# ilya16/MultINN

Measured on AMD Instinct MI355X. Metric: piano-roll timesteps/sec (train step), 5-track LSTM-NADE, higher is better.
Workload: dtype fp16; 1 GPU; TGT joint LSTM-NADE [1024,256,88,5]; global_batch=1024, per_gpu_batch=1024, seq_len=256, pitches=88, tracks=5, nade_hidden=256, optimizer=TF-Adam lr 0.01 eps 1e-4 clip 5.0, parallelism=dp1

## Files before the change

multinn_amd/csrc/nade_mfma.hip:

```cpp
#include "common.h"
typedef float nm_f4 __attribute__((ext_vector_type(4)));
#define NM_ST4(dst, a) __builtin_nontemporal_store((nm_f4){a[0], a[1], a[2], a[3]}, reinterpret_cast<nm_f4*>(dst))
#define NM_ST1(dst, x) __builtin_nontemporal_store((float)(x), dst)
#include <algorithm>
#include <type_traits>

typedef __bf16 bf16x8_t __attribute__((ext_vector_type(8)));
typedef float f32x4_t __attribute__((ext_vector_type(4)));
typedef __attribute__((address_space(1))) const void* gas_ptr_t;
typedef __attribute__((address_space(3))) void* lds_ptr_t;

#ifdef NM_TRACE
__device__ long long nm_trace[16];
#define NM_T(k) do { if (tid == 0 && blockIdx.x == NM_TRACE) { const long long now_ = wall_clock64(); nm_trace[k] += now_ - tprev_; tprev_ = now_; } } while (0)
#else
#define NM_T(k) do { } while (0)
#endif
#define NADE_EPS 1e-6f
#define LN2F 0.6931471805599453f
#define NM_H 256
#define NM_PITCH 264
#define NM_LP 36

__device__ __forceinline__ void lds_barrier() { asm volatile("s_waitcnt lgkmcnt(0)\n\ts_barrier" ::: "memory"); }

__device__ __forceinline__ float nm_ln(float x) { return __builtin_amdgcn_logf(x) * LN2F; }

typedef _Float16 f16x8_t __attribute__((ext_vector_type(8)));
struct NmPairB { f16x8_t hi, lo; };
template <bool SPLIT> struct NmState;
template <> struct NmState<false> { typedef bf16_t T; static constexpr int PITCH = NM_PITCH; };
template <> struct NmState<true> { typedef unsigned T; static constexpr int PITCH = 260; };
__device__ __forceinline__ unsigned nm_pack_hl(float x) {
    const float hi = __uint_as_float(__float_as_uint(x) & 0xFFFFE000u);
    return __builtin_bit_cast(unsigned, __builtin_amdgcn_cvt_pkrtz(hi, x - hi));
}

template <bool SPLIT>
struct NadeFwdSmemT {
    float sA[SPLIT ? 1 : 32][NM_H];
    typename NmState<SPLIT>::T sH[32][NmState<SPLIT>::PITCH];
    typename NmState<SPLIT>::T sF[32][NmState<SPLIT>::PITCH];
    float sLb[32][NM_LP];
    float sLf[32][NM_LP];
    unsigned sMask[2][32];
    unsigned sSb[2][33];
    unsigned short sFl[2][1024];
    unsigned short sPs[2][34];
    unsigned sAct[2][32];
};

__device__ __forceinline__ void nm_load_a(const bf16_t (*tile)[NM_PITCH], int mi, int lane, bf16x8_t (&a)[8]) {
    const bf16_t* p = &tile[16 * mi + (lane & 15)][8 * (lane >> 4)];
#pragma unroll
    for (int s = 0; s < 8; ++s) a[s] = *reinterpret_cast<const bf16x8_t*>(p + 32 * s);
}
template <bool SPLIT> __device__ __forceinline__ typename NmState<SPLIT>::T nm_state(float h) {
    if constexpr (SPLIT) return nm_pack_hl(h);
    else return f32_to_bf16(h);
}
__device__ __forceinline__ f32x4_t nm_dot(const bf16x8_t (&af)[8], const bf16x8_t (&bfr)[8]) {
    f32x4_t acc = {0.f, 0.f, 0.f, 0.f};
#pragma unroll
    for (int s = 0; s < 8; ++s) acc = __builtin_amdgcn_mfma_f32_16x16x32_bf16(af[s], bfr[s], acc, 0, 0, 0);
    return acc;
}
__device__ __forceinline__ f32x4_t nm_dot_hl(const unsigned (*tile)[260], int mi, int lane, const NmPairB (&bw)[8]) {
    const unsigned* p = &tile[16 * mi + (lane & 15)][8 * (lane >> 4)];
    f32x4_t accm = {0.f, 0.f, 0.f, 0.f}, accs = {0.f, 0.f, 0.f, 0.f};
#pragma unroll
    for (int s = 0; s < 8; ++s) {
        const uint4 q0 = *reinterpret_cast<const uint4*>(p + 32 * s), q1 = *reinterpret_cast<const uint4*>(p + 32 * s + 4);
        uint4 uh, ul;
        uh.x = __builtin_amdgcn_perm(q0.y, q0.x, 0x05040100u); ul.x = __builtin_amdgcn_perm(q0.y, q0.x, 0x07060302u);
        uh.y = __builtin_amdgcn_perm(q0.w, q0.z, 0x05040100u); ul.y = __builtin_amdgcn_perm(q0.w, q0.z, 0x07060302u);
        uh.z = __builtin_amdgcn_perm(q1.y, q1.x, 0x05040100u); ul.z = __builtin_amdgcn_perm(q1.y, q1.x, 0x07060302u);
        uh.w = __builtin_amdgcn_perm(q1.w, q1.z, 0x05040100u); ul.w = __builtin_amdgcn_perm(q1.w, q1.z, 0x07060302u);
        const f16x8_t ah = __builtin_bit_cast(f16x8_t, uh), al = __builtin_bit_cast(f16x8_t, ul);
        accs = __builtin_amdgcn_mfma_f32_16x16x32_f16(ah, bw[s].lo, accs, 0, 0, 0);
        accm = __builtin_amdgcn_mfma_f32_16x16x32_f16(ah, bw[s].hi, accm, 0, 0, 0);
        accs = __builtin_amdgcn_mfma_f32_16x16x32_f16(al, bw[s].hi, accs, 0, 0, 0);
    }
    return accm + accs;
}
template <bool SPLIT, typename Tile, typename B>
__device__ __forceinline__ void nm_logit_tile(const Tile& tile, int w, int lane, const B& bfr, float (*out)[NM_LP]) {
    const int ni = w >> 1, mi = w & 1;
    f32x4_t acc;
    if constexpr (SPLIT) {
        acc = nm_dot_hl(tile, mi, lane, bfr);
    } else {
        bf16x8_t af[8];
        nm_load_a(tile, mi, lane, af);
        acc = nm_dot(af, bfr);
    }
#pragma unroll
    for (int i = 0; i < 4; ++i) out[16 * mi + 4 * (lane >> 4) + i][16 * ni + (lane & 15)] = acc[i];
}

template <bool SPLIT>
__device__ __forceinline__ void
nade_fwd_mfma_body(int tracks, int N, int D, const uint8_t* __restrict__ v, long v_track_stride, const float* __restrict__ bias, int ld_bias,
                     const float* __restrict__ w_enc, const bf16_t* __restrict__ w_dec_bf, const float* __restrict__ row_weight,
                     float* __restrict__ nll, float* __restrict__ cond_p, float* __restrict__ d_bias, float* __restrict__ a_final,
                     const int* __restrict__ gate, int run_if, const int* __restrict__ n_rows_dev) {
    extern __shared__ __attribute__((aligned(16))) char smem_raw[];
    typedef NadeFwdSmemT<SPLIT> NadeFwdSmem;
    typedef typename NmState<SPLIT>::T state_t;
    typedef typename std::conditional<SPLIT, NmPairB, bf16x8_t>::type bfrag_t;
    constexpr int KS = 8;
    NadeFwdSmem& S = *reinterpret_cast<NadeFwdSmem*>(smem_raw);
    if (gate != nullptr && *gate != run_if) return;
    constexpr int Hn = NM_H;
    const int m = blockIdx.y;
    const int tid = threadIdx.x, lane = tid & 63, w = __builtin_amdgcn_readfirstlane(tid >> 6);
    const int ni = w >> 1;
    const int rb = blockIdx.x * 32;
    const uint8_t* __restrict__ vm = v + (size_t)m * v_track_stride;
    const float* __restrict__ we = w_enc + (size_t)m * D * Hn;
    const bf16_t* __restrict__ wd = w_dec_bf + (size_t)m * D * Hn * (SPLIT ? 2 : 1);
    const int bd_off = tracks * Hn + m * D;
    const int ntile = (D + 31) / 32;
    if (n_rows_dev != nullptr && rb >= *n_rows_dev) {
        if (d_bias != nullptr)
            for (int e = tid; e < 32 * D; e += 256) {
                const int n = e / D, i = e - n * D;
                if (rb + n < N) d_bias[(size_t)(rb + n) * ld_bias + bd_off + i] = 0.f;
            }
        if (nll != nullptr && tid < 32 && rb + tid < N) nll[(size_t)m * N + rb + tid] = 0.f;
        return;
    }

    float areg[SPLIT ? 32 : 1];
    {
        float av[32];
#pragma unroll
        for (int n = 0; n < 32; ++n) av[n] = bias[(size_t)min(rb + n, N - 1) * ld_bias + m * Hn + tid];
#pragma unroll
        for (int n = 0; n < 32; ++n) {
            const float x = rb + n < N ? av[n] : 0.f;
            if constexpr (SPLIT) areg[n] = x;
            else S.sA[n][tid] = x;
            S.sH[n][tid] = nm_state<SPLIT>(fast_sigmoid(x));
        }
    }
    auto load_v = [&](int c, unsigned char (&vb)[4]) {
#pragma unroll
        for (int i = 0; i < 4; ++i) {
            const int row = min(rb + 8 * w + 2 * i + (lane >> 5), N - 1), dd = min(32 * c + (lane & 31), D - 1);
            vb[i] = vm[(size_t)row * D + dd];
        }
    };
    auto ballots = [&](int c, const unsigned char (&vb)[4], unsigned (&msk)[32]) {
#pragma unroll
        for (int i = 0; i < 4; ++i) {
            const int row = rb + 8 * w + 2 * i + (lane >> 5), dd = 32 * c + (lane & 31);
            const unsigned long long bal = __ballot(row < N && dd < D && vb[i] != 0);
            if (lane == 0) { msk[8 * w + 2 * i] = (unsigned)bal; msk[8 * w + 2 * i + 1] = (unsigned)(bal >> 32); }
        }
    };
    auto build_list = [&](int buf) {
        if (w == 0) {
            const unsigned mk = lane < 32 ? S.sMask[buf][lane] : 0u;
            const int cnt = __popc(mk);
            unsigned rest = mk;
            int base = 0;
            for (int j = 0; j < 32; ++j) {
                const unsigned act = (unsigned)__ballot(cnt > j);
                if (lane == 0) { S.sPs[buf][j] = (unsigned short)base; S.sAct[buf][j] = act; }
                if (act == 0u) break;
                if (cnt > j) {
                    const int pos = base + __popc(act & ((1u << lane) - 1u));
                    const int dpos = __builtin_ctz(rest);
                    rest &= rest - 1;
                    S.sFl[buf][pos] = (unsigned short)((lane << 5) | dpos);
                }
                base += __popc(act);
            }
            if (lane == 0) S.sSb[buf][32] = (unsigned)base;
        }
    };
    auto load_b = [&](int c, bfrag_t (&b)[KS]) {
        const int d = min(32 * c + 16 * ni + (lane & 15), D - 1);
        if constexpr (SPLIT) {
            const f16_t* p = reinterpret_cast<const f16_t*>(wd) + (size_t)d * 2 * Hn + 8 * (lane >> 4);
#pragma unroll
            for (int s = 0; s < KS; ++s) {
                b[s].hi = *reinterpret_cast<const f16x8_t*>(p + 32 * s);
                b[s].lo = *reinterpret_cast<const f16x8_t*>(p + Hn + 32 * s);
            }
        } else {
            const bf16_t* p = wd + (size_t)d * Hn + 8 * (lane >> 4);
#pragma unroll
            for (int s = 0; s < KS; ++s) b[s] = *reinterpret_cast<const bf16x8_t*>(p + 32 * s);
        }
    };
    const __amdgpu_buffer_rsrc_t we_rs = __builtin_amdgcn_make_buffer_rsrc(const_cast<float*>(we), 0, D * Hn * 4, 0x00020000);
    auto load_we = [&](int c, int buf, int k0, float (&wv)[32]) {
        const int F = (int)S.sSb[buf][32];
        const int entv = (int)S.sFl[buf][(k0 + (lane & 31) < F) ? k0 + (lane & 31) : 0];
#pragma unroll
        for (int u = 0; u < 32; ++u) {
            const int e = __builtin_amdgcn_readlane(entv, u);
            wv[u] = __builtin_bit_cast(float, __builtin_amdgcn_raw_buffer_load_b32(we_rs, tid * 4, min(32 * c + (e & 31), D - 1) * (Hn * 4), 0));
        }
    };
    unsigned char vb[4];
    bfrag_t bfr[KS];
    float wev[32];
    load_v(0, vb);
    load_b(0, bfr);
    ballots(0, vb, S.sMask[0]);
    if (ntile > 1) load_v(1, vb);
    __syncthreads();
    build_list(0);
    __syncthreads();
    load_we(0, 0, 0, wev);

    const int en = tid >> 3, ed0 = 4 * (tid & 7), erow = rb + en;
    const bool evalid = erow < N;
    const int err = evalid ? erow : N - 1;
    const float rw = (row_weight != nullptr && evalid) ? row_weight[erow] : 0.f;
    float lp = 0.f;
#ifdef NM_TRACE
    long long tprev_ = wall_clock64();
#endif
    for (int c = 0; c < ntile; ++c) {
        const int buf = c & 1, nbuf = buf ^ 1;
        float bdec[4];
        {
            const float* bp = bias + (size_t)err * ld_bias + bd_off + 32 * c + ed0;
            if (32 * c + ed0 + 3 < D && (((size_t)bp) & 15) == 0) {
                const float4 b4 = *reinterpret_cast<const float4*>(bp);
                bdec[0] = b4.x; bdec[1] = b4.y; bdec[2] = b4.z; bdec[3] = b4.w;
            } else {
#pragma unroll
                for (int k = 0; k < 4; ++k) bdec[k] = bias[(size_t)err * ld_bias + bd_off + min(32 * c + ed0 + k, D - 1)];
            }
        }
        __builtin_amdgcn_sched_barrier(0);
        nm_logit_tile<SPLIT>(S.sH, w, lane, bfr, S.sLb);
        if (c + 1 < ntile) {
            ballots(c + 1, vb, S.sMask[nbuf]);
            if (c + 2 < ntile) load_v(c + 2, vb);
        }
        NM_T(0);
        lds_barrier();
        NM_T(1);
        const int F = (int)S.sSb[buf][32];
        const unsigned mk = S.sMask[buf][en];
        float lsel[4];
        int jj[4];
#pragma unroll
        for (int k = 0; k < 4; ++k) {
            jj[k] = __popc(mk & ((1u << (ed0 + k)) - 1u));
            lsel[k] = S.sLb[en][ed0 + k];
        }
        int slot_of[4];
#pragma unroll
        for (int k = 0; k < 4; ++k) {
            const int pj = max(jj[k] - 1, 0);
            slot_of[k] = jj[k] > 0 ? (int)S.sPs[buf][pj] + __popc(S.sAct[buf][pj] & ((1u << en) - 1u)) : -1;
        }
        for (int k0 = 0; k0 < F; k0 += 32) {
            if (k0 > 0) load_we(c, buf, k0, wev);
            const int cnt = min(32, F - k0);
            const int flv = (int)S.sFl[buf][min(k0 + (lane & 31), F - 1)];
#pragma unroll
            for (int u0 = 0; u0 < 32; u0 += 8) {
                if (u0 < cnt) {
                    int n[8];
#pragma unroll
                    for (int i = 0; i < 8; ++i) n[i] = __builtin_amdgcn_readlane(flv, u0 + i) >> 5;
                    if constexpr (SPLIT) {
                        float x[8];
#pragma unroll
                        for (int i = 0; i < 8; ++i) {
                            x[i] = areg[n[i]] + ((u0 + i < cnt) ? wev[u0 + i] : 0.f);
                            areg[n[i]] = x[i];
                        }
                        state_t hb[8];
#pragma unroll
                        for (int i = 0; i < 8; ++i) hb[i] = nm_state<SPLIT>(fast_sigmoid(x[i]));
#pragma unroll
                        for (int i = 0; i < 8; ++i) {
                            if (u0 + i < cnt) {
                                S.sF[u0 + i][tid] = hb[i];
                                S.sH[n[i]][tid] = hb[i];
                            }
                        }
                    } else {
                        bool indep = u0 + 8 <= cnt;
#pragma unroll
                        for (int i = 0; i < 7; ++i) indep = indep && n[i] < n[i + 1];
                        if (indep) {
                            float x[8];
#pragma unroll
                            for (int i = 0; i < 8; ++i) x[i] = S.sA[n[i]][tid];
#pragma unroll
                            for (int i = 0; i < 8; ++i) x[i] += wev[u0 + i];
                            state_t hb[8];
#pragma unroll
                            for (int i = 0; i < 8; ++i) hb[i] = nm_state<SPLIT>(fast_sigmoid(x[i]));
#pragma unroll
                            for (int i = 0; i < 8; ++i) {
                                S.sA[n[i]][tid] = x[i];
                                S.sF[u0 + i][tid] = hb[i];
                                S.sH[n[i]][tid] = hb[i];
                            }
                        } else {
#pragma unroll
                            for (int i = 0; i < 8; ++i) {
                                if (u0 + i < cnt) {
                                    const float av = S.sA[n[i]][tid] + wev[u0 + i];
                                    S.sA[n[i]][tid] = av;
                                    const state_t hb1 = nm_state<SPLIT>(fast_sigmoid(av));
                                    S.sF[u0 + i][tid] = hb1;
                                    S.sH[n[i]][tid] = hb1;
                                }
                            }
                        }
                    }
                }
            }
            NM_T(2);
            if (k0 == 0 && c + 1 < ntile) build_list(nbuf);
            NM_T(3);
            lds_barrier();
            NM_T(4);
            nm_logit_tile<SPLIT>(S.sF, w, lane, bfr, S.sLf);
            if (k0 == 0 && F <= 32 && c + 1 < ntile) load_we(c + 1, nbuf, 0, wev);
            NM_T(5);
            lds_barrier();
            NM_T(6);
#pragma unroll
            for (int k = 0; k < 4; ++k) {
                const int slot = slot_of[k] - k0;
                if (slot_of[k] >= 0 && slot >= 0 && slot < 32) lsel[k] = S.sLf[slot][ed0 + k];
            }
        }
        if (F == 0 && c + 1 < ntile) {
            build_list(nbuf);
            lds_barrier();
            load_we(c + 1, nbuf, 0, wev);
        } else if (F > 32 && c + 1 < ntile) {
            load_we(c + 1, nbuf, 0, wev);
        }
#pragma unroll
        for (int k = 0; k < 4; ++k) asm volatile("" :: "v"(bdec[k]));
        if (c + 1 < ntile) load_b(c + 1, bfr);
        NM_T(7);
        float prv[4], dbv[4];
#pragma unroll
        for (int k = 0; k < 4; ++k) {
            const int dpos = ed0 + k, gd = 32 * c + dpos;
            prv[k] = 0.f; dbv[k] = 0.f;
            if (gd >= D) continue;
            const float l = bdec[k] + lsel[k];
            const bool on = (mk >> dpos) & 1u;
            const float pr = fast_sigmoid(l);
            const float qr = fast_sigmoid(-l);
            lp += on ? nm_ln(NADE_EPS + pr) : nm_ln(NADE_EPS + qr);
            prv[k] = pr;
            const float dnll_dp = on ? -fast_rcp(NADE_EPS + pr) : fast_rcp(NADE_EPS + qr);
            dbv[k] = rw * dnll_dp * pr * qr;
        }
        if (evalid) {
            const int gd0 = 32 * c + ed0;
            const bool full = gd0 + 3 < D;
            if (cond_p != nullptr) {
                float* dst = cond_p + ((size_t)m * N + erow) * D + gd0;
                if (full && (((size_t)dst) & 15) == 0) NM_ST4(dst, prv);
                else {
#pragma unroll
                    for (int k = 0; k < 4; ++k) if (gd0 + k < D) dst[k] = prv[k];
                }
            }
            if (d_bias != nullptr) {
                float* dst = d_bias + (size_t)erow * ld_bias + bd_off + gd0;
                if (full && (((size_t)dst) & 15) == 0) NM_ST4(dst, dbv);
                else {
#pragma unroll
                    for (int k = 0; k < 4; ++k) if (gd0 + k < D) dst[k] = dbv[k];
                }
            }
        }
        NM_T(8);
    }
    lp += __shfl_xor(lp, 1);
    lp += __shfl_xor(lp, 2);
    lp += __shfl_xor(lp, 4);
    if ((tid & 7) == 0 && evalid && nll != nullptr) nll[(size_t)m * N + erow] = -lp;
    if (a_final != nullptr) {
#pragma unroll
        for (int n = 0; n < 32; ++n)
            if (rb + n < N) NM_ST1(&a_final[((size_t)m * N + rb + n) * Hn + tid], SPLIT ? areg[SPLIT ? n : 0] : S.sA[SPLIT ? 0 : n][tid]);
    }
}

template <bool SPLIT> __global__ void nade_fwd_mfma_kernel(int, int, int, const uint8_t*, long, const float*, int, const float*, const bf16_t*, const float*,
                                                           float*, float*, float*, float*, const int*, int, const int*);
template <>
__global__ void __launch_bounds__(256)
nade_fwd_mfma_kernel<false>(int tracks, int N, int D, const uint8_t* __restrict__ v, long v_track_stride, const float* __restrict__ bias, int ld_bias,
                            const float* __restrict__ w_enc, const bf16_t* __restrict__ w_dec_bf, const float* __restrict__ row_weight,
                            float* __restrict__ nll, float* __restrict__ cond_p, float* __restrict__ d_bias, float* __restrict__ a_final,
                            const int* __restrict__ gate, int run_if, const int* __restrict__ n_rows_dev) {
    nade_fwd_mfma_body<false>(tracks, N, D, v, v_track_stride, bias, ld_bias, w_enc, w_dec_bf, row_weight, nll, cond_p, d_bias, a_final, gate, run_if, n_rows_dev);
}
template <>
__global__ void __launch_bounds__(256) __attribute__((amdgpu_waves_per_eu(2, 2)))
nade_fwd_mfma_kernel<true>(int tracks, int N, int D, const uint8_t* __restrict__ v, long v_track_stride, const float* __restrict__ bias, int ld_bias,
                           const float* __restrict__ w_enc, const bf16_t* __restrict__ w_dec_bf, const float* __restrict__ row_weight,
                           float* __restrict__ nll, float* __restrict__ cond_p, float* __restrict__ d_bias, float* __restrict__ a_final,
                           const int* __restrict__ gate, int run_if, const int* __restrict__ n_rows_dev) {
    nade_fwd_mfma_body<true>(tracks, N, D, v, v_track_stride, bias, ld_bias, w_enc, w_dec_bf, row_weight, nll, cond_p, d_bias, a_final, gate, run_if, n_rows_dev);
}

extern "C" int mnn_nade_mfma_ok(int Hn) { return Hn == NM_H ? 1 : 0; }

extern "C" int mnn_nade_logprob_fwd_mfma(mnn_stream_t s, int tracks, int N, int D, int Hn, const uint8_t* v, long v_track_stride,
                                         const float* bias, int ld_bias, const float* w_enc, const void* w_dec_bf16, const float* row_weight,
                                         float* nll, float* cond_p, float* d_bias, float* a_final) {
    return mnn_nade_logprob_fwd_mfma_gated(s, tracks, N, D, Hn, v, v_track_stride, bias, ld_bias, w_enc, w_dec_bf16, row_weight, nll, cond_p, d_bias,
                                           a_final, nullptr, 0, nullptr);
}

template <bool SPLIT>
static int nm_launch(mnn_stream_t s, int tracks, int N, int D, int Hn, const uint8_t* v, long v_track_stride, const float* bias, int ld_bias,
                     const float* w_enc, const void* w_dec16, const float* row_weight, float* nll, float* cond_p, float* d_bias, float* a_final,
                     const int* gate, int run_if, const int* n_rows_dev) {
    MNN_REQUIRE(tracks > 0 && N > 0 && D > 0 && Hn == NM_H, "mnn_nade_logprob_fwd_mfma: need tracks,N,D>0 and Hn == 256 (Hn=%d)", Hn);
    MNN_REQUIRE(v && bias && w_enc && w_dec16, "mnn_nade_logprob_fwd_mfma: null pointer");
    MNN_REQUIRE(ld_bias >= tracks * (Hn + D), "mnn_nade_logprob_fwd_mfma: ld_bias %d < tracks*(Hn+D)", ld_bias);
    MNN_REQUIRE(d_bias == nullptr || row_weight != nullptr, "mnn_nade_logprob_fwd_mfma: d_bias needs row_weight");
    MNN_REQUIRE(((uintptr_t)w_dec16 & 15) == 0, "mnn_nade_logprob_fwd_mfma: the 16-bit decoder weights must be 16-byte aligned");
    static bool attr_set[64];
    int dev = 0;
    MNN_HIP(hipGetDevice(&dev));
    MNN_REQUIRE(dev >= 0 && dev < 64, "mnn_nade_logprob_fwd_mfma: device index %d", dev);
    if (!attr_set[dev]) {
        MNN_HIP(hipFuncSetAttribute((const void*)nade_fwd_mfma_kernel<SPLIT>, hipFuncAttributeMaxDynamicSharedMemorySize, (int)sizeof(NadeFwdSmemT<SPLIT>)));
        attr_set[dev] = true;
    }
    dim3 grid(cdiv(N, 32), tracks);
    hipLaunchKernelGGL(nade_fwd_mfma_kernel<SPLIT>, grid, dim3(256), sizeof(NadeFwdSmemT<SPLIT>), (hipStream_t)s, tracks, N, D, v, v_track_stride, bias,
                       ld_bias, w_enc, (const bf16_t*)w_dec16, row_weight, nll, cond_p, d_bias, a_final, gate, run_if, n_rows_dev);
    MNN_LAUNCH_CHECK();
    return MNN_OK;
}

extern "C" int mnn_nade_logprob_fwd_mfma_gated(mnn_stream_t s, int tracks, int N, int D, int Hn, const uint8_t* v, long v_track_stride,
                                               const float* bias, int ld_bias, const float* w_enc, const void* w_dec_bf16, const float* row_weight,
                                               float* nll, float* cond_p, float* d_bias, float* a_final, const int* gate, int run_if, const int* n_rows_dev) {
    return nm_launch<false>(s, tracks, N, D, Hn, v, v_track_stride, bias, ld_bias, w_enc, w_dec_bf16, row_weight, nll, cond_p, d_bias, a_final, gate, run_if, n_rows_dev);
}

extern "C" int mnn_nade_logprob_fwd_mfma_f32(mnn_stream_t s, int tracks, int N, int D, int Hn, const uint8_t* v, long v_track_stride,
                                             const float* bias, int ld_bias, const float* w_enc, const void* w_dec_packed, const float* row_weight,
                                             float* nll, float* cond_p, float* d_bias, float* a_final, const int* gate, int run_if, const int* n_rows_dev) {
    return nm_launch<true>(s, tracks, N, D, Hn, v, v_track_stride, bias, ld_bias, w_enc, w_dec_packed, row_weight, nll, cond_p, d_bias, a_final, gate, run_if, n_rows_dev);
}

__global__ void __launch_bounds__(256) nade_f32_pack_kernel(const float* __restrict__ w, long n, int Hn, float* __restrict__ out) {
    f16_t* o = reinterpret_cast<f16_t*>(out);
    for (long e = blockIdx.x * 256L + threadIdx.x; e < n; e += (long)gridDim.x * 256) {
        const long row = e / Hn;
        const int k = (int)(e - row * Hn);
        const float x = w[e];
        const f16_t hi = (f16_t)x;
        o[row * 2 * Hn + k] = hi;
        o[row * 2 * Hn + Hn + k] = (f16_t)(x - (float)hi);
    }
}
extern "C" int mnn_nade_f32_pack(mnn_stream_t s, const float* w_dec, long rows, int Hn, float* out) {
    MNN_REQUIRE(w_dec && out && rows > 0 && Hn > 0 && Hn % 8 == 0, "mnn_nade_f32_pack: bad arguments (Hn must be a multiple of 8)");
    MNN_REQUIRE(((uintptr_t)out & 15) == 0, "mnn_nade_f32_pack: the packed buffer must be 16-byte aligned");
    const long n = rows * Hn;
    hipLaunchKernelGGL(nade_f32_pack_kernel, dim3((int)std::min(2048L, (n + 255) / 256)), dim3(256), 0, (hipStream_t)s, w_dec, n, Hn, out);
    MNN_LAUNCH_CHECK();
    return MNN_OK;
}
```

Baseline: 20.05 million timesteps/s.

## Add 8-entry tail path for NADE tiles with 33-40 active units and parallelize list build

The active-pitch list builder is now spread across all four waves instead of running on wave 0 alone, with each wave writing every fourth step. Tiles with 33 to 40 active entries no longer run a second full 32-wide pass. They prefetch just 8 encoder weights and process the remainder in a short tail that runs the logit tile on half the waves, and the next tile's weight prefetch is moved earlier for them. Trace instrumentation is extended with atomic counters, but it is compiled only under NM_TRACE. The tail logic adds code complexity, and its correctness depends on the slot indexing staying consistent.

```diff
diff --git a/multinn_amd/csrc/nade_mfma.hip b/multinn_amd/csrc/nade_mfma.hip
--- a/multinn_amd/csrc/nade_mfma.hip
+++ b/multinn_amd/csrc/nade_mfma.hip
@@ -11,10 +11,13 @@
 typedef __attribute__((address_space(3))) void* lds_ptr_t;
 
 #ifdef NM_TRACE
-__device__ long long nm_trace[16];
-#define NM_T(k) do { if (tid == 0 && blockIdx.x == NM_TRACE) { const long long now_ = wall_clock64(); nm_trace[k] += now_ - tprev_; tprev_ = now_; } } while (0)
+__device__ unsigned long long nm_trace[24];
+#define NM_TRACED ((blockIdx.x & 63) == (NM_TRACE & 63))
+#define NM_T(k) do { if (tid == 0 && NM_TRACED) { const long long now_ = wall_clock64(); atomicAdd(&nm_trace[k], (unsigned long long)(now_ - tprev_)); tprev_ = now_; } } while (0)
+#define NM_COUNT(k, on) do { if (tid == 0 && (on)) atomicAdd(&nm_trace[k], 1ull); } while (0)
 #else
 #define NM_T(k) do { } while (0)
+#define NM_COUNT(k, on) do { } while (0)
 #endif
 #define NADE_EPS 1e-6f
 #define LN2F 0.6931471805599453f
@@ -160,25 +163,24 @@
         }
     };
     auto build_list = [&](int buf) {
-        if (w == 0) {
-            const unsigned mk = lane < 32 ? S.sMask[buf][lane] : 0u;
-            const int cnt = __popc(mk);
-            unsigned rest = mk;
-            int base = 0;
-            for (int j = 0; j < 32; ++j) {
-                const unsigned act = (unsigned)__ballot(cnt > j);
+        const unsigned mk = lane < 32 ? S.sMask[buf][lane] : 0u;
+        const int cnt = __popc(mk);
+        unsigned rest = mk;
+        int base = 0;
+        for (int j = 0; j < 32; ++j) {
+            const unsigned act = (unsigned)__ballot(cnt > j);
+            if ((j & 3) == w) {
                 if (lane == 0) { S.sPs[buf][j] = (unsigned short)base; S.sAct[buf][j] = act; }
-                if (act == 0u) break;
                 if (cnt > j) {
                     const int pos = base + __popc(act & ((1u << lane) - 1u));
-                    const int dpos = __builtin_ctz(rest);
-                    rest &= rest - 1;
-                    S.sFl[buf][pos] = (unsigned short)((lane << 5) | dpos);
-                }
-                base += __popc(act);
-            }
-            if (lane == 0) S.sSb[buf][32] = (unsigned)base;
-        }
+                    S.sFl[buf][pos] = (unsigned short)((lane << 5) | __builtin_ctz(rest));
+                }
+            }
+            if (act == 0u) break;
+            rest &= rest - 1;
+            base += __popc(act);
+        }
+        if (w == 0 && lane == 0) S.sSb[buf][32] = (unsigned)base;
     };
     auto load_b = [&](int c, bfrag_t (&b)[KS]) {
         const int d = min(32 * c + 16 * ni + (lane & 15), D - 1);
@@ -205,9 +207,18 @@
             wv[u] = __builtin_bit_cast(float, __builtin_amdgcn_raw_buffer_load_b32(we_rs, tid * 4, min(32 * c + (e & 31), D - 1) * (Hn * 4), 0));
         }
     };
+    auto load_we8 = [&](int c, int buf, float (&wv)[8]) {
+        const int F = (int)S.sSb[buf][32];
+        const int entv = (int)S.sFl[buf][(32 + (lane & 7) < F) ? 32 + (lane & 7) : 0];
+#pragma unroll
+        for (int u = 0; u < 8; ++u) {
+            const int e = __builtin_amdgcn_readlane(entv, u);
+            wv[u] = __builtin_bit_cast(float, __builtin_amdgcn_raw_buffer_load_b32(we_rs, tid * 4, min(32 * c + (e & 31), D - 1) * (Hn * 4), 0));
+        }
+    };
     unsigned char vb[4];
     bfrag_t bfr[KS];
-    float wev[32];
+    float wev[32], wev2[8];
     load_v(0, vb);
     load_b(0, bfr);
     ballots(0, vb, S.sMask[0]);
@@ -224,6 +235,7 @@
     float lp = 0.f;
 #ifdef NM_TRACE
     long long tprev_ = wall_clock64();
+    NM_COUNT(16, NM_TRACED);
 #endif
     for (int c = 0; c < ntile; ++c) {
         const int buf = c & 1, nbuf = buf ^ 1;
@@ -248,6 +260,7 @@
         lds_barrier();
         NM_T(1);
         const int F = (int)S.sSb[buf][32];
+        NM_COUNT(15, true); NM_COUNT(14, F > 32); NM_COUNT(18, F > 40); NM_COUNT(17, F > 32 && NM_TRACED);
         const unsigned mk = S.sMask[buf][en];
         float lsel[4];
         int jj[4];
@@ -262,7 +275,10 @@
             const int pj = max(jj[k] - 1, 0);
             slot_of[k] = jj[k] > 0 ? (int)S.sPs[buf][pj] + __popc(S.sAct[buf][pj] & ((1u << en) - 1u)) : -1;
         }
-        for (int k0 = 0; k0 < F; k0 += 32) {
+        const int Fu = __builtin_amdgcn_readfirstlane(F);
+        const bool tail8 = Fu > 32 && Fu <= 40;
+        if (tail8) load_we8(c, buf, wev2);
+        for (int k0 = 0; k0 < (tail8 ? 32 : F); k0 += 32) {
             if (k0 > 0) load_we(c, buf, k0, wev);
             const int cnt = min(32, F - k0);
             const int flv = (int)S.sFl[buf][min(k0 + (lane & 31), F - 1)];
@@ -323,29 +339,76 @@
                     }
                 }
             }
-            NM_T(2);
+            NM_T(k0 ? 9 : 2);
             if (k0 == 0 && c + 1 < ntile) build_list(nbuf);
             NM_T(3);
             lds_barrier();
-            NM_T(4);
+            NM_T(k0 ? 10 : 4);
             nm_logit_tile<SPLIT>(S.sF, w, lane, bfr, S.sLf);
-            if (k0 == 0 && F <= 32 && c + 1 < ntile) load_we(c + 1, nbuf, 0, wev);
-            NM_T(5);
+            if (k0 == 0 && (F <= 32 || tail8) && c + 1 < ntile) load_we(c + 1, nbuf, 0, wev);
+            NM_T(k0 ? 11 : 5);
             lds_barrier();
-            NM_T(6);
+            NM_T(k0 ? 12 : 6);
 #pragma unroll
             for (int k = 0; k < 4; ++k) {
                 const int slot = slot_of[k] - k0;
                 if (slot_of[k] >= 0 && slot >= 0 && slot < 32) lsel[k] = S.sLf[slot][ed0 + k];
             }
+        }
+        if (tail8) {
+            const int cnt = Fu - 32;
+            const int flv = (int)S.sFl[buf][min(32 + (lane & 7), F - 1)];
+            int n[8];
+#pragma unroll
+            for (int i = 0; i < 8; ++i) n[i] = __builtin_amdgcn_readlane(flv, i) >> 5;
+            if constexpr (SPLIT) {
+                float x[8];
+#pragma unroll
+                for (int i = 0; i < 8; ++i) {
+                    x[i] = areg[n[i]] + ((i < cnt) ? wev2[i] : 0.f);
+                    areg[n[i]] = x[i];
+                }
+                state_t hb[8];
+#pragma unroll
+                for (int i = 0; i < 8; ++i) hb[i] = nm_state<SPLIT>(fast_sigmoid(x[i]));
+#pragma unroll
+                for (int i = 0; i < 8; ++i) {
+                    if (i < cnt) {
+                        S.sF[i][tid] = hb[i];
+                        S.sH[n[i]][tid] = hb[i];
+                    }
+                }
+            } else {
+#pragma unroll
+                for (int i = 0; i < 8; ++i) {
+                    if (i < cnt) {
+                        const float av = S.sA[n[i]][tid] + wev2[i];
+                        S.sA[n[i]][tid] = av;
+                        const state_t hb1 = nm_state<SPLIT>(fast_sigmoid(av));
+                        S.sF[i][tid] = hb1;
+                        S.sH[n[i]][tid] = hb1;
+                    }
+                }
+            }
+            NM_T(9);
+            lds_barrier();
+            NM_T(10);
+            if ((w & 1) == 0) nm_logit_tile<SPLIT>(S.sF, w, lane, bfr, S.sLf);
+            NM_T(11);
+            lds_barrier();
+            NM_T(12);
+#pragma unroll
+            for (int k = 0; k < 4; ++k)
+                if (slot_of[k] >= 32) lsel[k] = S.sLf[slot_of[k] - 32][ed0 + k];
         }
         if (F == 0 && c + 1 < ntile) {
             build_list(nbuf);
             lds_barrier();
             load_we(c + 1, nbuf, 0, wev);
-        } else if (F > 32 && c + 1 < ntile) {
+        } else if (F > 40 && c + 1 < ntile) {
             load_we(c + 1, nbuf, 0, wev);
         }
+        if (F > 32) NM_T(13);
 #pragma unroll
         for (int k = 0; k < 4; ++k) asm volatile("" :: "v"(bdec[k]));
         if (c + 1 < ntile) load_b(c + 1, bfr);
```

Result: no change. 20.15 million timesteps/s, median of 6 (+0.5%).
